# Zhang-Xin-Duke/multimodal-detection-consistency

Measured on AMD Instinct MI355X. Metric: defended queries/sec, higher is better.
Workload: dtype bf16; 1 GPU; ViT-L/14 bf16, batch=512/GPU, N=8 variants, 1000000-row bf16 bank, encode + exact top-5 bank search + consistency (BASELINE configs[2]); global_batch=512, parallelism=dp1, text_packing=eot-packed + variant prefix sharing (bit-identical, see DESIGN.md), bank=gaussian + planted neighbours of the text rows

## Files before the change

### include/tvc.h

```cpp
#ifndef TVC_H_
#define TVC_H_

#include <stdint.h>

#ifdef __cplusplus
extern "C" {
#endif

#define TVC_ABI_VERSION 4
#define TVC_MAX_BANKS 8
#define TVC_MAX_TOPK 128

enum {
    TVC_OK = 0,
    TVC_E_INVALID = 1,
    TVC_E_HIP = 2,
    TVC_E_NOMEM = 3,
    TVC_E_STATE = 4,
    TVC_E_OVERFLOW = 5
};

enum { TVC_DTYPE_BF16 = 0, TVC_DTYPE_F32 = 1 };

typedef struct tvc_handle tvc_handle;
// ... 97 lines not shown
int tvc_encode_image(tvc_handle* h, const float* pix_dev, int32_t B,
                     float* out_dev, int32_t normalize, void* stream);

int tvc_encode_text(tvc_handle* h, const int32_t* tok_dev, int32_t T,
                    float* out_dev, int32_t normalize, void* stream);


int tvc_bank_select(tvc_handle* h, int32_t slot);

int tvc_bank_set(tvc_handle* h, const void* bank_dev, int64_t R, int32_t D,
                 int32_t dtype, void* stream);

int tvc_bank_search(tvc_handle* h, const float* rows_dev, int32_t M, int32_t k,
                    float count_thr, int64_t idx_offset,
                    int32_t* topk_idx_dev, float* topk_sim_dev, float* moments_dev,
                    void* stream);

int tvc_bank_search_dense(tvc_handle* h, const float* rows_dev, int32_t M, int32_t k,
                          float count_thr, int64_t idx_offset,
                          int32_t* topk_idx_dev, float* topk_sim_dev, float* moments_dev,
                          void* stream);

int tvc_bank_status(tvc_handle* h, void* stream);

int tvc_bank_gather(tvc_handle* h, const int32_t* idx_dev, int32_t n,
                    int64_t idx_offset, float* out_dev, void* stream);

int tvc_topk_merge(tvc_handle* h, const int32_t* idx_parts_dev, const float* sim_parts_dev,
                   const float* feat_parts_dev, const float* mom_parts_dev,
                   int32_t W, int32_t M, int32_t k, int32_t kf, int32_t D,
                   int32_t* idx_out_dev, float* sim_out_dev, float* feat_out_dev,
                   float* mom_out_dev, void* stream);



int tvc_kmeans_assign(tvc_handle* h, const float* centroids_dev, int32_t K,
                      int32_t* labels_dev, float* score_dev, float* dist2_dev, void* stream);

int tvc_kmeans_update(tvc_handle* h, const int32_t* labels_dev, const float* centroids_in_dev, int32_t K,
                      float* centroids_out_dev, int32_t* counts_dev, int32_t* offsets_dev, int32_t* order_dev,
                      void* stream);


#define TVC_RADIUS_MAX_ROWS 131072

int tvc_radius_graph(tvc_handle* h, float eps, uint32_t* adj_dev, int32_t* degree_dev, void* stream);
// ... 203 lines not shown
```

### multimodal-detection-consistency_amd/_lib.py

```python
from __future__ import annotations

import ctypes as C
import os
import subprocess
import threading
from pathlib import Path

PKG_DIR = Path(__file__).resolve().parent
CSRC_DIR = PKG_DIR / "csrc"
LIB_PATH = Path(os.environ["TVC_LIB_PATH"]) if os.environ.get("TVC_LIB_PATH") else PKG_DIR / "libtvc_hip.so"
HEADER_PATH = PKG_DIR.parent / "include" / "tvc.h"

TVC_OK, TVC_E_INVALID, TVC_E_HIP, TVC_E_NOMEM, TVC_E_STATE, TVC_E_OVERFLOW = range(6)
TVC_DTYPE_BF16, TVC_DTYPE_F32 = 0, 1
TVC_REC_HEAD, TVC_REC_MAXREF = 12, 16
TVC_ABI_VERSION, TVC_MAX_BANKS, TVC_MAX_TOPK = 4, 8, 128
TVC_OPT_TEXT_PACKING, TVC_OPT_MAX_CHUNK_IMAGES, TVC_OPT_MAX_CHUNK_TEXTS, TVC_OPT_BANK_FILTER = 1, 2, 3, 4
TVC_OPT_TEXT_GROUP = 5
TVC_OPT_POOLED_LAST_LAYER = 6
TVC_OPT_TOWER_PRECISION = 7
TVC_OPT_SD_ARENA_BYTES = 8
TVC_OPT_SD_STREAMS = 9
TVC_OPT_SD_PRECISION = 10
TVC_OPT_GRAD_PRECISION = 11
# ... 72 lines not shown

TOWER_OPS = {name: code for code, name in enumerate((
    "layernorm", "layernorm_bwd", "lnpre_bwd", "assemble_lnpre", "im2col", "im2col_f32", "col2im", "gelu_fwd", "gelu_bwd",
    "gelu_erf_16", "gelu_erf_f32", "l2norm_rows", "l2norm_bwd", "ln_split", "rows_split", "split_planes", "gather_rows",
    "gather_f32_rows", "text_lens_scan", "text_embed"))}

GRAD_SPLIT_OPS = {name: code for code, name in enumerate(("gelu_bwd", "l2norm_bwd", "lnpre_bwd", "rows_split_t", "layernorm_bwd"))}


SIGNATURES = {
    "tvc_abi_version": (C.c_uint32, []),
    "tvc_create": (C.c_int, [C.POINTER(ModelDesc), C.POINTER(VisionWeights), C.POINTER(TextWeights), C.POINTER(_P)]),
    "tvc_destroy": (None, [_P]),
    "tvc_last_error": (C.c_char_p, [_P]),
    "tvc_workspace_bytes": (C.c_uint64, [_P]),
    "tvc_set_option": (C.c_int, [_P, C.c_int32, C.c_int64]),
    "tvc_encode_image": (C.c_int, [_P, _P, C.c_int32, _P, C.c_int32, _P]),
    "tvc_encode_text": (C.c_int, [_P, _P, C.c_int32, _P, C.c_int32, _P]),
    "tvc_bank_set": (C.c_int, [_P, _P, C.c_int64, C.c_int32, C.c_int32, _P]),
    "tvc_bank_select": (C.c_int, [_P, C.c_int32]),
    "tvc_bank_search": (C.c_int, [_P, _P, C.c_int32, C.c_int32, C.c_float, C.c_int64, _P, _P, _P, _P]),
    "tvc_bank_search_dense": (C.c_int, [_P, _P, C.c_int32, C.c_int32, C.c_float, C.c_int64, _P, _P, _P, _P]),
    "tvc_bank_status": (C.c_int, [_P, _P]),
    "tvc_bank_gather": (C.c_int, [_P, _P, C.c_int32, C.c_int64, _P, _P]),
    "tvc_kmeans_assign": (C.c_int, [_P, _P, C.c_int32, _P, _P, _P, _P]),
    "tvc_kmeans_update": (C.c_int, [_P, _P, _P, C.c_int32, _P, _P, _P, _P, _P]),
    "tvc_radius_graph": (C.c_int, [_P, C.c_float, _P, _P, _P]),
    "tvc_dbscan_sweep": (C.c_int, [_P, _P, _P, C.c_int32, C.c_int32, _P, _P, C.c_int32, _P]),
    "tvc_dbscan_finish": (C.c_int, [_P, _P, _P, C.c_int32, C.c_int32, _P, _P, _P, _P, _P]),
    "tvc_graph_pair_count": (C.c_int, [_P, _P, C.c_int32, _P, _P, _P]),
    "tvc_graph_pair_fill": (C.c_int, [_P, _P, C.c_int32, _P, _P, _P, C.c_int64, _P]),
    "tvc_pair_cosine": (C.c_int, [_P, _P, C.c_int64, _P, _P]),
    "tvc_ivf_probe": (C.c_int, [_P, _P, C.c_int32, C.c_int32, _P, C.c_int32, C.c_int32, _P, _P, _P]),
    "tvc_ivf_scan": (C.c_int, [_P, _P, C.c_int32, C.c_int32, _P, C.c_int32, _P, C.c_int32, C.c_int32, _P, C.c_int64, _P, _P, _P, _P]),
    "tvc_topk_merge": (C.c_int, [_P, _P, _P, _P, _P, C.c_int32, C.c_int32, C.c_int32, C.c_int32, C.c_int32,
                                 _P, _P, _P, _P, _P]),
    "tvc_cosine_matrix": (C.c_int, [_P, _P, C.c_int32, _P, C.c_int32, C.c_int32, _P, _P]),
    "tvc_consistency": (C.c_int, [_P, _P, _P, C.c_int32, C.c_int32, C.c_int32, _P, _P, _P, C.c_int32, C.c_int32,
                                  C.POINTER(ConsistencyParams), _P, _P]),
    "tvc_profile_begin": (C.c_int, [_P]),
    "tvc_profile_end": (C.c_int, [_P, C.POINTER(C.c_double), C.POINTER(C.c_double), C.POINTER(C.c_int64), _P]),
    "tvc_gemm_bf16": (C.c_int, [_P, _P, _P, _P, _P, C.c_int32, C.c_int32, C.c_int32, C.c_int64, C.c_int64, C.c_int32,
                                C.c_int32, _P]),
    "tvc_attention": (C.c_int, [_P, _P, _P, C.c_int32, C.c_int32, C.c_int32, C.c_int32, _P]),
    "tvc_layernorm": (C.c_int, [_P, _P, _P, _P, _P, C.c_int32, C.c_int32, _P]),
    "tvc_encode_text_hidden": (C.c_int, [_P, _P, C.c_int32, _P, _P]),
# ... 83 lines not shown
```

### multimodal-detection-consistency_amd/csrc/bank.hip

```cpp
#include "gemm_core.hpp"
#include "gemm_ring4.hpp"
#include "skinny.hpp"
#include "kernels.hpp"
#include "launch.hpp"
#include "select.hpp"
#include <cstdlib>

#define BANK_POOL 6144
#define BANK_MAX_RESCORE_D 2048
#define BANK_LDS_BYTES (GEMM_LDS_BYTES + 256 * 4 + 2 * 256 * 4 * 4)

struct Cand {
    float v;
    int32_t idx;
};

struct Moments {
    float sum = 0.f, sq = 0.f, mx = -INFINITY, cnt = 0.f;
};
__device__ __forceinline__ Moments combine(const Moments a, const Moments b) {
    Moments r;
    r.sum = a.sum + b.sum; r.sq = a.sq + b.sq; r.mx = fmaxf(a.mx, b.mx); r.cnt = a.cnt + b.cnt;
    return r;
}
__device__ __forceinline__ Moments mom_load(const float* p) {
    Moments r;
    r.sum = p[0]; r.sq = p[1]; r.mx = p[2]; r.cnt = p[3];
    return r;
}
__device__ __forceinline__ void mom_store(float* p, const Moments m) { p[0] = m.sum; p[1] = m.sq; p[2] = m.mx; p[3] = m.cnt; }
template <int... Os>
__device__ __forceinline__ Moments mom_lanes(Moments m) {
    ((m.sum += __shfl_xor(m.sum, Os, 64)), ...);
    ((m.sq += __shfl_xor(m.sq, Os, 64)), ...);
    ((m.cnt += __shfl_xor(m.cnt, Os, 64)), ...);
    ((m.mx = fmaxf(m.mx, __shfl_xor(m.mx, Os, 64))), ...);
    return m;
}


__device__ __forceinline__ void kth_finish(float m, int q, int k, float* __restrict__ tau, const uint16_t* __restrict__ qplanes,
                                           int D, const float* __restrict__ bank_bounds, float* gm, float (*nrm)[4]) {
    const int t = threadIdx.x;
    float margin = 0.f;
    if (qplanes) {
        float h2 = 0.f, l2 = 0.f;
        if (t < 256) {
            const uint16_t* qr = qplanes + (int64_t)q * 2 * D;
            for (int c = t; c < D; c += 256) {
                const float h = bf16_bits_to_f32(qr[c]), l = bf16_bits_to_f32(qr[D + c]);
                h2 = fmaf(h, h, h2); l2 = fmaf(l, l, l2);
            }
            h2 = wave_sum(h2); l2 = wave_sum(l2);
            if ((t & 63) == 0) { nrm[0][t >> 6] = h2; nrm[1][t >> 6] = l2; }
        }
        __syncthreads();
        const float qh = sqrtf(nrm[0][0] + nrm[0][1] + nrm[0][2] + nrm[0][3]);
        const float ql = sqrtf(nrm[1][0] + nrm[1][1] + nrm[1][2] + nrm[1][3]);
        const float bh = bank_bounds[0], bl = bank_bounds[1];
        margin = (bh * ql + bl * qh + bl * ql) * 1.001f + 4e-6f * (1.f + bh * qh);
    }
    if (t < 256) gm[t] = m;
    __syncthreads();
    if (t >= 256) return;
    int rank = 0;
    for (int u = 0; u < 256; ++u) {
        const float o = gm[u];
        rank += (o > m) || (o == m && u < t);
    }
    const int keff = k > BANK_KEFF ? k : BANK_KEFF;
    if (rank == keff - 1) {
        float v = m;
        if (v > -INFINITY) v = v - 1e-6f - 1e-6f * fabsf(v) - margin;
        if (!(v == v)) v = -INFINITY;
        tau[q] = v;
    }
}

__global__ __launch_bounds__(1024) void kth_bound_kernel(const float* __restrict__ s0, int n_sample,
                                                         int k, float* __restrict__ tau,
                                                         const uint16_t* __restrict__ qplanes, int D,
                                                         const float* __restrict__ bank_bounds) {
    __shared__ float gm[256];
    __shared__ float part[3][256];
    __shared__ float nrm[2][4];
    const int q = blockIdx.x, t = threadIdx.x;
    const float* row = s0 + (int64_t)q * n_sample;
    float m = -INFINITY;
    if ((n_sample & 3) == 0) {
        const f32x4_t* row4 = (const f32x4_t*)row;
        const int n4 = n_sample >> 2;
        int i = t;
        for (; i + 3 * 1024 < n4; i += 4 * 1024) {
            const f32x4_t a = row4[i], b = row4[i + 1024], c = row4[i + 2048], d = row4[i + 3072];
            m = fmaxf(m, fmaxf(fmaxf(fmaxf(a[0], a[1]), fmaxf(a[2], a[3])), fmaxf(fmaxf(b[0], b[1]), fmaxf(b[2], b[3]))));
            m = fmaxf(m, fmaxf(fmaxf(fmaxf(c[0], c[1]), fmaxf(c[2], c[3])), fmaxf(fmaxf(d[0], d[1]), fmaxf(d[2], d[3]))));
        }
        for (; i < n4; i += 1024) {
            const f32x4_t a = row4[i];
            m = fmaxf(m, fmaxf(fmaxf(a[0], a[1]), fmaxf(a[2], a[3])));
        }
    } else {
        for (int i = t; i < n_sample; i += 1024) m = fmaxf(m, row[i]);
    }
    if (t >= 256) part[(t >> 8) - 1][t & 255] = m;
    __syncthreads();
    if (t < 256) m = fmaxf(fmaxf(m, part[0][t]), fmaxf(part[1][t], part[2][t]));
    kth_finish(m, q, k, tau, qplanes, D, bank_bounds, gm, nrm);
}

__global__ __launch_bounds__(256) void kth_groups_kernel(const float* __restrict__ gmax, int k, float* __restrict__ tau,
                                                         const uint16_t* __restrict__ qplanes, int D,
                                                         const float* __restrict__ bank_bounds, int32_t* __restrict__ overflow) {
    __shared__ float gm[256];
    __shared__ float nrm[2][4];
    const int q = blockIdx.x;
    if (q == 0 && threadIdx.x == 0) *overflow = 0;
    kth_finish(gmax[(int64_t)q * 256 + threadIdx.x], q, k, tau, qplanes, D, bank_bounds, gm, nrm);
}

__global__ __launch_bounds__(256) void bank_bounds_kernel(BankRows bank, uint32_t* __restrict__ out_sq) {
    const int lane = threadIdx.x & 63, D = bank.D;
    float mh = 0.f, ml = 0.f;
    for (int64_t r = (int64_t)blockIdx.x * 4 + (threadIdx.x >> 6); r < bank.R; r += (int64_t)gridDim.x * 4) {
        const uint16_t* br = bank.p + r * bank.ld;
        float h2 = 0.f, l2 = 0.f;
        for (int c = lane * 8; c < D; c += 512) {
            const u32x4_t h = *(const u32x4_t*)(br + c);
#pragma unroll
            for (int e = 0; e < 4; ++e) {
                const float a = Op16<false>::lo(h[e]), b = Op16<false>::hi(h[e]);
                h2 = fmaf(a, a, fmaf(b, b, h2));
            }
            if (bank.planes > 1) {
                const u32x4_t l = *(const u32x4_t*)(br + D + c);
#pragma unroll
                for (int e = 0; e < 4; ++e) {
                    const float a = Op16<false>::lo(l[e]), b = Op16<false>::hi(l[e]);
                    l2 = fmaf(a, a, fmaf(b, b, l2));
                }
            }
// ... 342 lines not shown

template <int KB>
static hipError_t launch_sample_skinny_kb(const uint16_t* bank, int64_t ldb, const uint16_t* qplanes, int M, int n_sample,
                                          int sample_stride, float* gmax, hipStream_t stream) {
    const int nqt = M <= 16 ? 1 : (M > 32 && M <= 48) ? 3 : 2;
    const int per = (n_sample + 255) / 256;
    const dim3 grid(256, (M + nqt * 16 - 1) / (nqt * 16));
    const size_t lds = (size_t)nqt * 16 * (KB * 256 + 16) + 8 * nqt * 16 * 4;
    return dispatch<1, 2, 3>(nqt, [&](auto n) {
        constexpr size_t max_lds = n.value * 16 * (KB * 256 + 16) + 8 * n.value * 16 * 4;
        return launch<bank_sample_skinny_kernel<KB, n.value>, max_lds>(grid, dim3(512), lds, stream, bank, ldb, qplanes, M, n_sample,
                                                                       sample_stride, per, gmax);
    });
}
static hipError_t launch_bank_sample_skinny(const uint16_t* bank, int64_t ldb, int D, const uint16_t* qplanes, int M, int n_sample,
                                            int sample_stride, float* gmax, hipStream_t stream) {
    return dispatch<128, 512, 768>(D, [&](auto d) {
        return launch_sample_skinny_kb<d.value / 64>(bank, ldb, qplanes, M, n_sample, sample_stride, gmax, stream);
    });
}

#define SEL_T 1024
#define SEL_W (SEL_T / 64)
#define SEL_CPT 8
__global__ __launch_bounds__(SEL_T) void bank_select_kernel(const Cand* __restrict__ cand,
                                                            const int32_t* __restrict__ cand_cnt,
                                                            const float* __restrict__ mom_part, int S, int M,
                                                            int k, int32_t* __restrict__ topk_idx,
                                                            float* __restrict__ topk_sim,
                                                            float* __restrict__ moments,
                                                            int32_t* __restrict__ overflow, BankRows rs,
                                                            const float* __restrict__ rs_rows,
                                                            int64_t idx_offset) {
    __shared__ Cand pool[BANK_POOL];
    __shared__ __attribute__((aligned(16))) float qs[BANK_MAX_RESCORE_D];
    __shared__ int wsum[SEL_W];
    __shared__ BestSlots<SEL_T, 1> red;
    __shared__ float mom_red[SEL_W][4];
    const int q = blockIdx.x, t = threadIdx.x, D = rs.D;
    const int lane = t & 63, wave = t >> 6;

    const bool few = S <= SEL_T * SEL_CPT;
    int cnt[SEL_CPT];
    int mine = 0;
    if (few) {
#pragma unroll
        for (int u = 0; u < SEL_CPT; ++u) {
            const int c = t + u * SEL_T;
            cnt[u] = c < S ? cand_cnt[(int64_t)c * M + q] : 0;
        }
#pragma unroll
        for (int u = 0; u < SEL_CPT; ++u) mine += cnt[u];
    } else {
        for (int c = t; c < S; c += SEL_T) mine += cand_cnt[(int64_t)c * M + q];
    }
    int total_all;
    int off = block_exclusive_scan<SEL_T>(mine, wsum, total_all);
    if (few) {
#pragma unroll
        for (int u = 0; u < SEL_CPT; ++u) {
            const int n = cnt[u];
            if (n > 0) {
                const Cand* src = cand + ((int64_t)(t + u * SEL_T) * M + q) * BANK_CAP;
                for (int i = 0; i < n; ++i) {
                    if (off < BANK_POOL) pool[off] = src[i];
                    ++off;
                }
            }
        }
    } else {
        for (int c = t; c < S; c += SEL_T) {
            const int n = cand_cnt[(int64_t)c * M + q];
            const Cand* src = cand + ((int64_t)c * M + q) * BANK_CAP;
            for (int i = 0; i < n; ++i) {
                if (off < BANK_POOL) pool[off] = src[i];
                ++off;
            }
        }
    }
    if (t == 0 && total_all > BANK_POOL) atomicOr(overflow, 2);
    const int total = total_all < BANK_POOL ? total_all : BANK_POOL;
    if (rs.p) {
        for (int c = t; c < D; c += SEL_T) qs[c] = rs_rows[(int64_t)q * D + c];
    }
    __syncthreads();

    if (rs.p) {
        for (int i0 = wave; i0 < total; i0 += 4 * SEL_W) {
            float part[4];
            const uint16_t* br[4];
#pragma unroll
            for (int u = 0; u < 4; ++u) {
                int i = i0 + u * SEL_W;
                i = i < total ? i : total - 1;
                br[u] = rs.p + ((int64_t)pool[i].idx - idx_offset) * rs.ld;
                part[u] = 0.f;
            }
            for (int c = lane * 8; c < D; c += 512) {
                u32x4_t h[4], l[4];
#pragma unroll
                for (int u = 0; u < 4; ++u) {
                    h[u] = *(const u32x4_t*)(br[u] + c);
                    if (rs.planes > 1) l[u] = *(const u32x4_t*)(br[u] + D + c);
                }
                const f32x4_t q0 = *(const f32x4_t*)(qs + c), q1 = *(const f32x4_t*)(qs + c + 4);
#pragma unroll
                for (int u = 0; u < 4; ++u) {
#pragma unroll
                    for (int e2 = 0; e2 < 4; ++e2) {
                        float a = Op16<false>::lo(h[u][e2]), b = Op16<false>::hi(h[u][e2]);
                        if (rs.planes > 1) {
                            a += Op16<false>::lo(l[u][e2]);
                            b += Op16<false>::hi(l[u][e2]);
                        }
                        const float qa = e2 < 2 ? q0[e2 * 2] : q1[e2 * 2 - 4];
                        const float qb = e2 < 2 ? q0[e2 * 2 + 1] : q1[e2 * 2 - 3];
                        part[u] = fmaf(a, qa, fmaf(b, qb, part[u]));
                    }
                }
            }
#pragma unroll
            for (int u = 0; u < 4; ++u) {
                const float v = wave_sum(part[u]);
                const int i = i0 + u * SEL_W;
                if (lane == 0 && i < total) pool[i].v = v;
            }
        }
        __syncthreads();
    }

    for (int r = 0; r < k; ++r) {
        Best<1> b;
        b.pay[0] = -1;
        for (int i = t; i < total; i += SEL_T) {
            const Cand c = pool[i];
            if (c.idx >= 0) best_take(b, Best<1>{c.v, c.idx, {i}});
        }
        const Best<1> f = block_best(b, red, r);
        const int fp = f.pay[0];
        if (t == 0) {
            topk_idx[(int64_t)q * k + r] = fp >= 0 ? f.id : -1;
            topk_sim[(int64_t)q * k + r] = fp >= 0 ? f.v : -INFINITY;
        }
        if (fp >= 0 && (fp & (SEL_T - 1)) == t) pool[fp].idx = -1;
    }

    if (moments) {
        Moments m;
        for (int ch = t; ch < S; ch += SEL_T) m = combine(m, mom_load(mom_part + ((int64_t)ch * M + q) * 4));
        m = mom_lanes<32, 16, 8, 4, 2, 1>(m);
        if (lane == 0) mom_store(mom_red[wave], m);
        __syncthreads();
        if (t == 0) {
            Moments o;
            for (int w = 0; w < SEL_W; ++w) o = combine(o, mom_load(mom_red[w]));
            mom_store(moments + (int64_t)q * 4, o);
        }
// ... 52 lines not shown
        if (st != hipSuccess) return st;
    }
    return hipSuccess;
}

static bool env_flag(const char* name) {
    const char* v = getenv(name);
    return !v || atoi(v) != 0;
}

hipError_t launch_bank_search(const BankSearchLaunch& L, hipStream_t stream) {
    const BankRows& B = L.bank;
    const int D = B.D;
    const bool filter = (L.moments == nullptr) && L.bank_bounds && L.rows && D <= BANK_MAX_RESCORE_D && L.allow_filter;

    static const bool skinny_on = env_flag("TVC_BANK_SKINNY");
    const bool skinny = filter && skinny_on && skinny_covers(D, L.M) && B.ld % 8 == 0;
    static const bool skinny_sample_on = env_flag("TVC_BANK_SKINNY_SAMPLE");

    hipError_t st;
    if (skinny && skinny_sample_on && B.planes == 1) {
        st = launch_bank_sample_skinny(B.p, B.ld, D, L.qplanes, L.M, L.n_sample, L.sample_stride, L.gmax, stream);
        if (st != hipSuccess) return st;
        st = launch<kth_groups_kernel>(dim3(L.M), dim3(256), 0, stream, L.gmax, L.k, L.tau, L.qplanes, D, L.bank_bounds, L.overflow);
        if (st != hipSuccess) return st;
    } else {
        const GemmLaunch G = gemm_launch_planes(B.p, B.ld * (int64_t)L.sample_stride, L.n_sample, B.planes, L.qplanes, L.M, D,
                                                L.s0, L.n_sample);
        st = launch_gemm_bf16(G, stream);
        if (st != hipSuccess) return st;
        st = launch<kth_bound_kernel>(dim3(L.M), dim3(1024), 0, stream, L.s0, L.n_sample, L.k, L.tau, filter ? L.qplanes : nullptr, D,
                                      L.bank_bounds);
        if (st != hipSuccess) return st;
        st = hipMemsetAsync(L.overflow, 0, sizeof(int32_t), stream);
        if (st != hipSuccess) return st;
    }

    GemmOperands g = gemm_operands(gemm_launch_planes(B.p, B.ld, (int)B.R, B.planes, L.qplanes, L.M, D, nullptr, 0));
    if (filter) g.planes = 1;
    BankEpilogue e;
    e.tau = L.tau; e.cand = (Cand*)L.cand; e.cand_cnt = L.cand_cnt; e.mom_part = L.mom_part;
    e.overflow = L.overflow; e.R = B.R; e.idx_offset = L.idx_offset; e.M = L.M; e.count_thr = L.count_thr;
    const int nQt = (L.M + GEMM_BN - 1) / GEMM_BN;
    const int nbt = (int)((B.R + GEMM_BM - 1) / GEMM_BM);
    const int tpc = (nbt + L.S - 1) / L.S;
    static const bool ring_on = env_flag("TVC_BANK_RING");
    const bool ring = filter && ring_on && L.q_rows_padded && (g.lda % 64 == 0) && (g.ldb % 64 == 0) && B.R >= GEMM_BM;
    const dim3 grid(nQt * L.S), block(GEMM_THREADS);
    if (skinny)
        st = launch_bank_filter_skinny(B.p, B.ld, D, L.qplanes, e, L.S, tpc * GEMM_BM, stream);
    else if (ring)
        st = launch<bank_filter_ring_kernel, BANK_LDS_BYTES>(grid, block, BANK_LDS_BYTES, stream, g, e, nQt, L.S, tpc, nbt);
    else
        st = dispatch<false, true>(filter, [&](auto f) {
            return launch<bank_search_kernel<f.value>, BANK_LDS_BYTES>(grid, block, BANK_LDS_BYTES, stream, g, e, nQt, L.S, tpc, nbt);
        });
    if (st != hipSuccess) return st;

    BankRows rs = B;
    if (!filter) rs.p = nullptr;
    return launch<bank_select_kernel>(dim3(L.M), dim3(SEL_T), 0, stream, (const Cand*)L.cand, L.cand_cnt, L.mom_part, L.S, L.M, L.k,
                                      L.topk_idx, L.topk_sim, L.moments, L.overflow, rs, L.rows, L.idx_offset);
}

__global__ __launch_bounds__(256) void topk_merge_kernel(const int32_t* __restrict__ idx_parts,
                                                         const float* __restrict__ sim_parts,
                                                         const float* __restrict__ feat_parts,
                                                         const float* __restrict__ mom_parts, int W,
                                                         int M, int k, int kf, int D,
                                                         int32_t* __restrict__ idx_out,
                                                         float* __restrict__ sim_out,
                                                         float* __restrict__ feat_out,
                                                         float* __restrict__ mom_out) {
    __shared__ float sv[256];
    __shared__ int si[256];
    __shared__ int src_of_rank[32];
    const int q = blockIdx.x, t = threadIdx.x;
    const int n = W * k;
    float v = -INFINITY;
    int id = -1;
    if (t < n) {
        const int w = t / k, j = t - w * k;
        id = idx_parts[((int64_t)w * M + q) * k + j];
        v = (id >= 0) ? sim_parts[((int64_t)w * M + q) * k + j] : -INFINITY;
    }
// ... 56 lines not shown
```

### multimodal-detection-consistency_amd/csrc/handle.hpp

```cpp
#pragma once
#include "../../include/tvc.h"
#include "kernels.hpp"

#include <hip/hip_runtime.h>
#include <cstdio>
#include <cstring>
#include <string>
#include <vector>

inline thread_local std::string g_create_error;

enum Slot {
    WS_X = 0, WS_H, WS_QKV, WS_MLP, WS_CLS, WS_DELTA, WS_DELTA2, WS_SPLITK, WS_POOL, WS_TOWER_N,
    WS_TX = WS_TOWER_N, WS_TH, WS_TQKV, WS_TMLP, WS_TCLS, WS_TDELTA, WS_TDELTA2, WS_TSPLITK, WS_TPOOL,
    WS_PATCH, WS_EOT, WS_STARTS, WS_PFX, WS_LENS,
    WS_COSX, WS_COSY, WS_COSXP, WS_COSYP,
    WS_QPLANES, WS_S0, WS_TAU, WS_CAND, WS_CAND_CNT, WS_MOM_PART, WS_OVERFLOW,
    WS_GSAVE, WS_GOUT, WS_GXL, WS_GDX, WS_G16, WS_GMLP2, WS_GDQKV, WS_GSTATS, WS_GSMALL, WS_GPATCH,
    WS_PX, WS_PH, WS_PQKV, WS_PMLP, WS_PCLS, WS_P_N_END,
    WS_PTX = WS_P_N_END, WS_PTH, WS_PTQKV, WS_PTMLP, WS_PTCLS,
    WS_SX, WS_SH, WS_SQKV, WS_SU, WS_SM, WS_SDELTA1, WS_SDELTA2, WS_SCLS, WS_S_END,
    WS_STX = WS_S_END, WS_STH, WS_STQKV, WS_STU, WS_STM, WS_STDELTA1, WS_STDELTA2, WS_STCLS,
    WS_SD0, WS_SD1, WS_SD2, WS_SD3, WS_SD4, WS_SD5, WS_SD6, WS_SD7,
    WS_KM_CPLANES, WS_KM_HALFNORM, WS_KM_BLKCNT, WS_KM_OFFSETS, WS_KM_ORDER,
    WS_IVF_CPLANES, WS_IVF_PQPLANES, WS_IVF_HALFNORM, WS_IVF_SIMS,
    WS_IVF_QPLANES, WS_IVF_BLKCNT, WS_IVF_PCOUNTS, WS_IVF_POFFSETS, WS_IVF_PORDER, WS_IVF_SCORES,
    WS_GS_KEEP, WS_GS_GP, WS_GS_MP, WS_GS_WIDE, WS_GS_ROW, WS_GS_SMALL,
    WS_DB_NORM2, WS_DB_HALF,
    WS_COUNT
};

struct Buf {
    void* p = nullptr;
    size_t n = 0;
};

struct BankSlot {
    const uint16_t* bank = nullptr;
    void* owned = nullptr;
    int64_t R = 0;
// ... 19 lines not shown
    int gI = 0, gJ = 0, gK = 0, gP = 0, gS = 0;
};

template <class W, class L>
struct TowerWeights {
    W w{};
    std::vector<L> layers;
    bool set = false;
    void assign(const W& src, int n_layers) {
        w = src;
        layers.assign(src.layers, src.layers + n_layers);
        w.layers = layers.data();
        set = true;
    }
};

struct tvc_handle {
    tvc_model_desc desc{};
    TowerWeights<tvc_vision_weights, tvc_layer_weights> vision;
    TowerWeights<tvc_text_weights, tvc_layer_weights> text;
    BankSlot banks[TVC_MAX_BANKS];
    int cur_bank = 0;
    bool bank_filter = true;
    Buf ws[WS_COUNT];
    std::string err;
    int max_chunk_images = 512;
    int max_chunk_texts = 4608;
    bool pack_text = true;
    int text_group = 0;
    bool pooled_last = true;
    std::vector<void*> wT;
    int grad_B = 0;
    int grad_normalize = 0;
    const float* grad_pix = nullptr;
    int grad_precision = 0;
    int grad_mode = 0;
    bool prof = false;
    std::vector<ProfRec> prof_recs;
    TowerWeights<tvc_vision_weights_f32, tvc_layer_weights_f32> vision32;
    TowerWeights<tvc_text_weights_f32, tvc_layer_weights_f32> text32;
    int tower_precision = 0;
    TowerWeights<tvc_vision_weights, tvc_layer_weights> vision16;
    TowerWeights<tvc_text_weights, tvc_layer_weights> text16;
    std::vector<SplitLayer> vsplit, tsplit;
    uint16_t* vsplit_patch = nullptr;
    std::vector<void*> split_owned;
// ... 119 lines not shown
```

### multimodal-detection-consistency_amd/csrc/kernels.hpp

```cpp
#pragma once
#include <hip/hip_runtime.h>
#include <stdint.h>
#include "host_plan.hpp"

struct BankRows {
    const uint16_t* p = nullptr;
    int64_t ld = 0;
    int64_t R = 0;
    int D = 0;
    int planes = 1;
};

enum { TVC_EPI_F32 = 0, TVC_EPI_BF16 = 1, TVC_EPI_GELU_BF16 = 2, TVC_EPI_RESID_F32 = 3 };

struct GemmLaunch {
    const uint16_t* A = nullptr;
    const uint16_t* B = nullptr;
    int64_t lda = 0, ldb = 0;
    int I = 0, J = 0, K = 0;
    int planes = 1;
    int a_plane_off[9] = {0, 0, 0, 0, 0, 0, 0, 0, 0};
    int b_plane_off[9] = {0, 0, 0, 0, 0, 0, 0, 0, 0};
    bool splitk_small = false;
    int splitk_fixed = 0;
// ... 53 lines not shown
hipError_t launch_split_planes(const float* x, uint16_t* out, int64_t rows, int d, int planes,
                               hipStream_t stream);
hipError_t launch_gather_rows(const BankRows& bank, const int32_t* idx, int64_t idx_offset, int n, float* out, hipStream_t stream);

hipError_t launch_attention(const uint16_t* qkv, uint16_t* out, const int32_t* starts, int n_seq,
                            int seq_len, int heads, int causal, hipStream_t stream, const int32_t* pfx = nullptr,
                            int pool_mode = 0, const int32_t* pool_row = nullptr,
                            int f16 = 0);

struct BankSearchLaunch {
    BankRows bank;
    const uint16_t* qplanes = nullptr;
    const float* rows = nullptr;
    const float* bank_bounds = nullptr;
    bool allow_filter = true;
    bool q_rows_padded = false;
    int M = 0;
    int k = 0;
    float count_thr = 0.f;
    int64_t idx_offset = 0;
    float* s0 = nullptr;
    float* gmax = nullptr;
    float* tau = nullptr;
    void* cand = nullptr;
    int32_t* cand_cnt = nullptr;
    float* mom_part = nullptr;
    int32_t* overflow = nullptr;
    int n_sample = 0, sample_stride = 1, S = 0, cap = 0;
    int32_t* topk_idx = nullptr;
    float* topk_sim = nullptr;
    float* moments = nullptr;
};
hipError_t launch_bank_search(const BankSearchLaunch& L, hipStream_t stream);
hipError_t launch_bank_bounds(const BankRows& bank, float* bounds, hipStream_t stream);
hipError_t launch_bank_search_dense(const BankSearchLaunch& L, float* sims_ws, int block_rows, hipStream_t stream);
hipError_t launch_topk_merge(const int32_t* idx_parts, const float* sim_parts, const float* feat_parts,
                             const float* mom_parts, int W, int M, int k, int kf, int D,
                             int32_t* idx_out, float* sim_out, float* feat_out, float* mom_out,
                             hipStream_t stream);

struct KmeansAssignLaunch {
    BankRows bank;
    const float* centroids = nullptr;
    const uint16_t* cplanes = nullptr;
    int K = 0;
    float* halfnorm = nullptr;
// ... 172 lines not shown
```

### multimodal-detection-consistency_amd/csrc/tvc_abi.cpp

```cpp
#include "handle.hpp"

#include <cstdlib>

namespace {

bool tower_ok(const tvc_tower_arch& a) {
    return a.width > 0 && a.layers > 0 && a.heads > 0 && a.width == a.heads * 64 && a.width % 64 == 0 &&
           a.width <= 1024 && a.mlp > 0 && a.mlp % 64 == 0 && (a.act == TVC_ACT_QUICK_GELU || a.act == TVC_ACT_GELU);
}

struct PoolBufs { uint16_t *Hc, *D1c, *H2c, *MLPc, *D2c; };
PoolBufs pool_bufs(tvc_handle* h, const tvc_tower_arch& a, int n_seq, int wso) {
    uint16_t* p = (uint16_t*)h->ws[WS_POOL + wso].p;
    const size_t nd = ((size_t)n_seq + 256) * a.width;
    PoolBufs b;
    b.Hc = p; b.D1c = p + nd; b.H2c = p + 2 * nd; b.D2c = p + 3 * nd; b.MLPc = p + 4 * nd;
    return b;
}
size_t pool_bytes(const tvc_tower_arch& a, int n_seq) {
    return (((size_t)n_seq + 256) * a.width * 4 + ((size_t)n_seq + 256) * a.mlp) * 2;
}

struct GradSave {
    float* x;
// ... 378 lines not shown
                    int64_t idx_offset, int32_t* topk_idx_dev, float* topk_sim_dev, float* moments_dev,
                    void* stream) {
    if (!h) return TVC_E_INVALID;
    BankSlot& bk = h->banks[h->cur_bank];
    if (!bk.bank && bk.R != 0) return fail(h, TVC_E_STATE, "tvc_bank_search: no bank registered");
    if (bk.D == 0) return fail(h, TVC_E_STATE, "tvc_bank_search: call tvc_bank_set first");
    if (M < 0 || k < 1 || k > TVC_MAX_TOPK || (M > 0 && (!rows_dev || !topk_idx_dev || !topk_sim_dev)))
        return fail(h, TVC_E_INVALID, "tvc_bank_search: need 1 <= k <= 128 and non-NULL buffers");
    if (M == 0) return TVC_OK;
    hipStream_t st = (hipStream_t)stream;
    const int D = bk.D;
    if (bk.R == 0) {
        HIP_TRY(hipMemsetAsync(topk_idx_dev, 0xff, (size_t)M * k * 4, st));
        HIP_TRY(hipMemsetAsync(topk_sim_dev, 0, (size_t)M * k * 4, st));
        if (moments_dev) HIP_TRY(hipMemsetAsync(moments_dev, 0, (size_t)M * 16, st));
        return TVC_OK;
    }
    BankSearchLaunch L;
    bank_plan(bk.R, M, k, &L.n_sample, &L.sample_stride, &L.S, &L.cap);
    int rc;
    if ((rc = ensure(h, WS_QPLANES, (size_t)((M + 255) / 256 * 256) * 2 * D * 2))) return rc;
    if ((rc = ensure(h, WS_S0, (size_t)M * (L.n_sample > 256 ? L.n_sample : 256) * 4))) return rc;
    if ((rc = ensure(h, WS_TAU, (size_t)M * 4))) return rc;
    if ((rc = ensure(h, WS_CAND, (size_t)L.S * M * L.cap * 8))) return rc;
    if ((rc = ensure(h, WS_CAND_CNT, (size_t)L.S * M * 4))) return rc;
    if ((rc = ensure(h, WS_MOM_PART, (size_t)L.S * M * 16))) return rc;
    if ((rc = ensure(h, WS_OVERFLOW, 16))) return rc;
    HIP_TRY(launch_split_planes(rows_dev, (uint16_t*)h->ws[WS_QPLANES].p, M, D, 2, st));
    L.bank = bank_rows(bk);
    L.qplanes = (const uint16_t*)h->ws[WS_QPLANES].p; L.q_rows_padded = true; L.M = M; L.k = k; L.count_thr = count_thr;
    L.idx_offset = idx_offset;
    L.rows = rows_dev; L.bank_bounds = bk.bounds; L.allow_filter = h->bank_filter;
    L.s0 = (float*)h->ws[WS_S0].p; L.gmax = L.s0; L.tau = (float*)h->ws[WS_TAU].p; L.cand = h->ws[WS_CAND].p;
    L.cand_cnt = (int32_t*)h->ws[WS_CAND_CNT].p; L.mom_part = (float*)h->ws[WS_MOM_PART].p;
    L.overflow = (int32_t*)h->ws[WS_OVERFLOW].p;
    L.topk_idx = topk_idx_dev; L.topk_sim = topk_sim_dev; L.moments = moments_dev;
    {
        const bool filter = !moments_dev && h->bank_filter && D <= 2048;
        const int planes = filter ? 1 : bank_products(bk.planes);
        ProfScope ps(h, st, TVC_PROF_BANK, 2.0 * (double)bk.R * M * D * planes);
        HIP_TRY(launch_bank_search(L, st));
    }
    return TVC_OK;
}

int tvc_bank_search_dense(tvc_handle* h, const float* rows_dev, int32_t M, int32_t k, float count_thr,
                          int64_t idx_offset, int32_t* topk_idx_dev, float* topk_sim_dev, float* moments_dev,
                          void* stream) {
    if (!h) return TVC_E_INVALID;
    BankSlot& bk = h->banks[h->cur_bank];
    if (bk.D == 0 || (!bk.bank && bk.R != 0)) return fail(h, TVC_E_STATE, "tvc_bank_search_dense: call tvc_bank_set first");
    if (M < 0 || k < 1 || k > TVC_MAX_TOPK || (M > 0 && (!rows_dev || !topk_idx_dev || !topk_sim_dev)))
        return fail(h, TVC_E_INVALID, "tvc_bank_search_dense: need 1 <= k <= 128 and non-NULL buffers");
    if (M == 0) return TVC_OK;
    if (bk.R == 0) return tvc_bank_search(h, rows_dev, M, k, count_thr, idx_offset, topk_idx_dev, topk_sim_dev, moments_dev, stream);
    hipStream_t st = (hipStream_t)stream;
    const int D = bk.D;
    int block = (int)((size_t)1 << 28) / (int)(bk.R > 0 ? bk.R : 1);
    if (block > 64) block = 64;
    if (block < 1) block = 1;
    int rc;
    if ((rc = ensure(h, WS_QPLANES, (size_t)((M + 255) / 256 * 256) * 2 * D * 2))) return rc;
    if ((rc = ensure(h, WS_S0, (size_t)block * bk.R * 4))) return rc;
    HIP_TRY(launch_split_planes(rows_dev, (uint16_t*)h->ws[WS_QPLANES].p, M, D, 2, st));
    BankSearchLaunch L;
// ... 280 lines not shown
                           int32_t seq_len, int32_t heads, void* stream) {
    if (!h) return TVC_E_INVALID;
    if (!qkv_dev || !dout_dev || !dqkv_dev) return fail(h, TVC_E_INVALID, "tvc_attention_backward: NULL buffer");
    if (n_seq < 0 || seq_len < 0 || heads < 0)
        return fail(h, TVC_E_INVALID, "tvc_attention_backward: n_seq, seq_len and heads must not be negative");
    int rc;
    if ((rc = ensure(h, WS_GSTATS, (size_t)n_seq * seq_len * heads * 16))) return rc;
    HIP_TRY(launch_attention_bwd(qkv_dev, dout_dev, dqkv_dev, (float*)h->ws[WS_GSTATS].p, n_seq, seq_len, heads, (hipStream_t)stream));
    return TVC_OK;
}

int tvc_layernorm_backward(tvc_handle* h, const float* x_dev, const uint16_t* dy_dev, const float* g_dev, const float* dres_dev,
                           float* dx_dev, int32_t rows, int32_t d, void* stream) {
    if (!h) return TVC_E_INVALID;
    if (!x_dev || !dy_dev || !g_dev || !dx_dev) return fail(h, TVC_E_INVALID, "tvc_layernorm_backward: NULL buffer");
    HIP_TRY(launch_layernorm_bwd(x_dev, d, nullptr, dy_dev, 0, g_dev, dres_dev, dx_dev, nullptr, rows, d, d, (hipStream_t)stream));
    return TVC_OK;
}

int tvc_set_option(tvc_handle* h, int32_t option, int64_t value) {
    if (!h) return TVC_E_INVALID;
    switch (option) {
        case TVC_OPT_TEXT_PACKING: h->pack_text = value != 0; return TVC_OK;
        case TVC_OPT_BANK_FILTER: h->bank_filter = value != 0; return TVC_OK;
        case TVC_OPT_POOLED_LAST_LAYER: h->pooled_last = value != 0; return TVC_OK;
        case TVC_OPT_TOWER_PRECISION: {
            if (value < 0 || value > 3)
                return fail(h, TVC_E_INVALID, "tvc_set_option: TVC_OPT_TOWER_PRECISION must be 0 (bf16), 1 (fp32), 2 (split-bf16) or 3 (fp16)");
            if (value == 3) {
                if (!h->vision16.set && !h->text16.set)
                    return fail(h, TVC_E_INVALID, "tvc_set_option: TVC_OPT_TOWER_PRECISION = 3 needs tvc_set_weights_f16 first");
                h->tower_precision = 3; return TVC_OK;
            }
            if (value != 0 && !h->vision32.set && !h->text32.set)
                return fail(h, TVC_E_STATE, "tvc_set_option: TVC_OPT_TOWER_PRECISION = 1 / 2 needs tvc_set_weights_f32 first");
            if (value == 2) {
                const int rc = tvc_split_prepare(h);
                if (rc) return rc;
            }
            h->tower_precision = (int)value; return TVC_OK;
        }
        case TVC_OPT_GRAD_PRECISION:
            if (value != 0 && value != 2)
                return fail(h, TVC_E_INVALID, "tvc_set_option: TVC_OPT_GRAD_PRECISION must be 0 (bf16) or 2 (split-bf16)");
            if (value == 2 && h->vision32.set) {
                const int rc = tvc_split_prepare(h);
                if (rc) return rc;
// ... 168 lines not shown
```

### multimodal-detection-consistency_amd/engine.py

```python
from __future__ import annotations

import contextlib
import ctypes as C
import threading
from dataclasses import dataclass, field
from typing import Dict, Optional, Tuple

import torch

from . import _lib
from .arch import ClipArch


@dataclass
class ConsistencyConfig:
    reference_count: int = 5
    similarity_threshold: float = 0.3
    retrieval_top_k: int = 10
    dup_threshold: float = 0.95
    w_text_variants: float = 0.4
    w_consistency: float = 0.2
    w_exp: Tuple[float, float, float, float] = (0.25, 0.25, 0.25, 0.25)
    search_k: int = 5

# ... 439 lines not shown
        self.dense_fallbacks += 1
        return out

    def bank_search_dense(self, rows: torch.Tensor, k: int, count_thr: float = 0.3, idx_offset: int = 0,
                          want_moments: bool = True, bank: str = DEFAULT_BANK, out=None):
        if not 1 <= k <= _lib.TVC_MAX_TOPK:
            raise ValueError(f"top-k must be in [1, {_lib.TVC_MAX_TOPK}] (got {k})")
        rows = _require_cuda(rows, torch.float32, "rows")
        M = rows.shape[0]
        if out is None:
            out = (torch.empty((M, k), dtype=torch.int32, device=self.device),
                   torch.empty((M, k), dtype=torch.float32, device=self.device),
                   torch.empty((M, 4), dtype=torch.float32, device=self.device) if want_moments else None)
        idx, sim, mom = out
        with self._lock, torch.cuda.device(self.device):
            self._select(bank)
            self._check(self.lib.tvc_bank_search_dense(self.handle, _ptr(rows), M, k, count_thr, idx_offset,
                                                       _ptr(idx), _ptr(sim), _ptr(mom), _stream()))
        return idx, sim, mom

    def bank_status(self) -> None:
        with self._lock, torch.cuda.device(self.device):
            self._check(self.lib.tvc_bank_status(self.handle, _stream()))

    def bank_gather(self, idx: torch.Tensor, idx_offset: int = 0, bank: str = DEFAULT_BANK) -> torch.Tensor:
        idx = _require_cuda(idx, torch.int32, "idx")
        n = idx.numel()
        with self._lock, torch.cuda.device(self.device):
            b = self._select(bank)
            out = torch.empty((n, b["dim"]), dtype=torch.float32, device=self.device)
            self._check(self.lib.tvc_bank_gather(self.handle, _ptr(idx), n, idx_offset, _ptr(out), _stream()))
        return out.view(*idx.shape, b["dim"])

    def kmeans_assign(self, centroids: torch.Tensor, bank: str = DEFAULT_BANK):
        centroids = _require_cuda(centroids, torch.float32, "centroids")
        with self._lock, torch.cuda.device(self.device):
            b = self._select(bank)
            if centroids.dim() != 2 or centroids.shape[1] != b["dim"]:
                raise ValueError(f"centroids must be [K, {b['dim']}] (got {tuple(centroids.shape)})")
            R = b["rows"]
            labels = torch.empty(R, dtype=torch.int32, device=self.device)
            score = torch.empty(R, dtype=torch.float32, device=self.device)
            dist2 = torch.empty(R, dtype=torch.float32, device=self.device)
            self._check(self.lib.tvc_kmeans_assign(self.handle, _ptr(centroids), centroids.shape[0], _ptr(labels), _ptr(score),
                                                   _ptr(dist2), _stream()))
        return labels, score, dist2
# ... 587 lines not shown
```

Baseline: 5305 queries/s.

## Prune rescore candidates with a bounded error band before exact bank rescoring

The select kernel now finds the approximate k-th best score in the candidate pool. It then drops every candidate whose approximate score falls below that value minus an error band built from the per-query quantisation margin and bf16 rounding slack, and compacts the pool before the exact two-plane rescore. The aim is to cut the global bank-row reads and dot products spent in the rescore pass. In exchange it adds k block-wide reductions, a scan, and new margin and live-count buffers, along with a debug API to read the live counts. Rows per rescore iteration drop from 4 to 2, with an occupancy hint in launch bounds.

```diff
diff --git a/include/tvc.h b/include/tvc.h
--- a/include/tvc.h
+++ b/include/tvc.h
@@ -143,6 +143,8 @@
                           void* stream);
 
 int tvc_bank_status(tvc_handle* h, void* stream);
+
+int tvc_bank_live_counts(tvc_handle* h, int32_t* out_dev, int32_t M, void* stream);
 
 int tvc_bank_gather(tvc_handle* h, const int32_t* idx_dev, int32_t n,
                     int64_t idx_offset, float* out_dev, void* stream);
diff --git a/multimodal-detection-consistency_amd/_lib.py b/multimodal-detection-consistency_amd/_lib.py
--- a/multimodal-detection-consistency_amd/_lib.py
+++ b/multimodal-detection-consistency_amd/_lib.py
@@ -118,6 +118,7 @@
     "tvc_bank_search": (C.c_int, [_P, _P, C.c_int32, C.c_int32, C.c_float, C.c_int64, _P, _P, _P, _P]),
     "tvc_bank_search_dense": (C.c_int, [_P, _P, C.c_int32, C.c_int32, C.c_float, C.c_int64, _P, _P, _P, _P]),
     "tvc_bank_status": (C.c_int, [_P, _P]),
+    "tvc_bank_live_counts": (C.c_int, [_P, _P, C.c_int32, _P]),
     "tvc_bank_gather": (C.c_int, [_P, _P, C.c_int32, C.c_int64, _P, _P]),
     "tvc_kmeans_assign": (C.c_int, [_P, _P, C.c_int32, _P, _P, _P, _P]),
     "tvc_kmeans_update": (C.c_int, [_P, _P, _P, C.c_int32, _P, _P, _P, _P, _P]),
diff --git a/multimodal-detection-consistency_amd/csrc/bank.hip b/multimodal-detection-consistency_amd/csrc/bank.hip
--- a/multimodal-detection-consistency_amd/csrc/bank.hip
+++ b/multimodal-detection-consistency_amd/csrc/bank.hip
@@ -40,7 +40,8 @@
 
 
 __device__ __forceinline__ void kth_finish(float m, int q, int k, float* __restrict__ tau, const uint16_t* __restrict__ qplanes,
-                                           int D, const float* __restrict__ bank_bounds, float* gm, float (*nrm)[4]) {
+                                           int D, const float* __restrict__ bank_bounds, float* gm, float (*nrm)[4],
+                                           float* __restrict__ margin_out) {
     const int t = threadIdx.x;
     float margin = 0.f;
     if (qplanes) {
@@ -59,6 +60,7 @@
         const float ql = sqrtf(nrm[1][0] + nrm[1][1] + nrm[1][2] + nrm[1][3]);
         const float bh = bank_bounds[0], bl = bank_bounds[1];
         margin = (bh * ql + bl * qh + bl * ql) * 1.001f + 4e-6f * (1.f + bh * qh);
+        if (t == 0 && margin_out) margin_out[q] = margin;
     }
     if (t < 256) gm[t] = m;
     __syncthreads();
@@ -80,7 +82,7 @@
 __global__ __launch_bounds__(1024) void kth_bound_kernel(const float* __restrict__ s0, int n_sample,
                                                          int k, float* __restrict__ tau,
                                                          const uint16_t* __restrict__ qplanes, int D,
-                                                         const float* __restrict__ bank_bounds) {
+                                                         const float* __restrict__ bank_bounds, float* __restrict__ margin_out) {
     __shared__ float gm[256];
     __shared__ float part[3][256];
     __shared__ float nrm[2][4];
@@ -106,17 +108,18 @@
     if (t >= 256) part[(t >> 8) - 1][t & 255] = m;
     __syncthreads();
     if (t < 256) m = fmaxf(fmaxf(m, part[0][t]), fmaxf(part[1][t], part[2][t]));
-    kth_finish(m, q, k, tau, qplanes, D, bank_bounds, gm, nrm);
+    kth_finish(m, q, k, tau, qplanes, D, bank_bounds, gm, nrm, margin_out);
 }
 
 __global__ __launch_bounds__(256) void kth_groups_kernel(const float* __restrict__ gmax, int k, float* __restrict__ tau,
                                                          const uint16_t* __restrict__ qplanes, int D,
-                                                         const float* __restrict__ bank_bounds, int32_t* __restrict__ overflow) {
+                                                         const float* __restrict__ bank_bounds, int32_t* __restrict__ overflow,
+                                                         float* __restrict__ margin_out) {
     __shared__ float gm[256];
     __shared__ float nrm[2][4];
     const int q = blockIdx.x;
     if (q == 0 && threadIdx.x == 0) *overflow = 0;
-    kth_finish(gmax[(int64_t)q * 256 + threadIdx.x], q, k, tau, qplanes, D, bank_bounds, gm, nrm);
+    kth_finish(gmax[(int64_t)q * 256 + threadIdx.x], q, k, tau, qplanes, D, bank_bounds, gm, nrm, margin_out);
 }
 
 __global__ __launch_bounds__(256) void bank_bounds_kernel(BankRows bank, uint32_t* __restrict__ out_sq) {
@@ -505,8 +508,11 @@
 
 #define SEL_T 1024
 #define SEL_W (SEL_T / 64)
-#define SEL_CPT 8
-__global__ __launch_bounds__(SEL_T) void bank_select_kernel(const Cand* __restrict__ cand,
+#define SEL_ROWS 2
+#define SEL_CPT 2
+#define SEL_OWN (BANK_POOL / SEL_T)
+static_assert(SEL_OWN * SEL_T == BANK_POOL && (SEL_T & (SEL_T - 1)) == 0, "the pool is dealt evenly to the threads");
+__global__ __launch_bounds__(SEL_T, 8) void bank_select_kernel(const Cand* __restrict__ cand,
                                                             const int32_t* __restrict__ cand_cnt,
                                                             const float* __restrict__ mom_part, int S, int M,
                                                             int k, int32_t* __restrict__ topk_idx,
@@ -514,10 +520,13 @@
                                                             float* __restrict__ moments,
                                                             int32_t* __restrict__ overflow, BankRows rs,
                                                             const float* __restrict__ rs_rows,
-                                                            int64_t idx_offset) {
+                                                            int64_t idx_offset, const float* __restrict__ margin,
+                                                            const float* __restrict__ bank_bounds,
+                                                            int32_t* __restrict__ live_out) {
     __shared__ Cand pool[BANK_POOL];
     __shared__ __attribute__((aligned(16))) float qs[BANK_MAX_RESCORE_D];
     __shared__ int wsum[SEL_W];
+    __shared__ float qn2[SEL_W];
     __shared__ BestSlots<SEL_T, 1> red;
     __shared__ float mom_red[SEL_W][4];
     const int q = blockIdx.x, t = threadIdx.x, D = rs.D;
@@ -564,31 +573,86 @@
     if (t == 0 && total_all > BANK_POOL) atomicOr(overflow, 2);
     const int total = total_all < BANK_POOL ? total_all : BANK_POOL;
     if (rs.p) {
-        for (int c = t; c < D; c += SEL_T) qs[c] = rs_rows[(int64_t)q * D + c];
-    }
-    __syncthreads();
+        float q2 = 0.f;
+        for (int c = t; c < D; c += SEL_T) {
+            const float x = rs_rows[(int64_t)q * D + c];
+            qs[c] = x;
+            q2 = fmaf(x, x, q2);
+        }
+        q2 = wave_sum(q2);
+        if (lane == 0) qn2[wave] = q2;
+    }
+    __syncthreads();
+
+    int n_live = total;
+    if (rs.p && margin) {
+        float qn = 0.f;
+#pragma unroll
+        for (int w = 0; w < SEL_W; ++w) qn += qn2[w];
+        qn = sqrtf(qn);
+        const float slack = 1.01f * (3.f * (float)D * 5.9604645e-8f + 3.0517578e-5f) * (bank_bounds[0] + bank_bounds[1]) * qn;
+        const float band = 2.f * (margin[q] + slack);
+        bool prune = total_all <= BANK_POOL && total >= k && band < INFINITY;
+        Cand own[SEL_OWN];
+#pragma unroll
+        for (int j = 0; j < SEL_OWN; ++j) {
+            const int i = t + j * SEL_T;
+            own[j].v = -INFINITY; own[j].idx = -1;
+            if (i < total) own[j] = pool[i];
+        }
+        unsigned struck = 0u;
+        float L = 0.f;
+        for (int r = 0; prune && r < k; ++r) {
+            Best<1> b;
+            b.pay[0] = -1;
+#pragma unroll
+            for (int j = 0; j < SEL_OWN; ++j)
+                if (own[j].idx >= 0 && !((struck >> j) & 1u)) best_take(b, Best<1>{own[j].v, own[j].idx, {t + j * SEL_T}});
+            const Best<1> f = block_best(b, red, r);
+            const int fp = f.pay[0];
+            if (fp < 0) prune = false;
+            else if ((fp & (SEL_T - 1)) == t) struck |= 1u << (fp / SEL_T);
+            L = f.v;
+        }
+        if (prune) {
+            float thr = L - band;
+            thr -= 4.8e-7f * fabsf(thr);
+            int mine_live = 0;
+#pragma unroll
+            for (int j = 0; j < SEL_OWN; ++j) {
+                if (!(own[j].idx >= 0 && own[j].v >= thr)) own[j].idx = -1;
+                mine_live += own[j].idx >= 0 ? 1 : 0;
+            }
+            int at = block_exclusive_scan<SEL_T>(mine_live, wsum, n_live);
+#pragma unroll
+            for (int j = 0; j < SEL_OWN; ++j)
+                if (own[j].idx >= 0) pool[at++] = own[j];
+        }
+        __syncthreads();
+    }
+    if (live_out && t == 0) { live_out[2 * (int64_t)q] = n_live; live_out[2 * (int64_t)q + 1] = total; }
 
     if (rs.p) {
-        for (int i0 = wave; i0 < total; i0 += 4 * SEL_W) {
-            float part[4];
-            const uint16_t* br[4];
-#pragma unroll
-            for (int u = 0; u < 4; ++u) {
+        for (int i0 = wave; i0 < n_live; i0 += SEL_ROWS * SEL_W) {
+            float part[SEL_ROWS];
+            const uint16_t* br[SEL_ROWS];
+#pragma unroll
+            for (int u = 0; u < SEL_ROWS; ++u) {
                 int i = i0 + u * SEL_W;
-                i = i < total ? i : total - 1;
+                i = i < n_live ? i : n_live - 1;
                 br[u] = rs.p + ((int64_t)pool[i].idx - idx_offset) * rs.ld;
                 part[u] = 0.f;
             }
             for (int c = lane * 8; c < D; c += 512) {
-                u32x4_t h[4], l[4];
-#pragma unroll
-                for (int u = 0; u < 4; ++u) {
+                u32x4_t h[SEL_ROWS], l[SEL_ROWS];
+#pragma unroll
+                for (int u = 0; u < SEL_ROWS; ++u) {
                     h[u] = *(const u32x4_t*)(br[u] + c);
                     if (rs.planes > 1) l[u] = *(const u32x4_t*)(br[u] + D + c);
                 }
                 const f32x4_t q0 = *(const f32x4_t*)(qs + c), q1 = *(const f32x4_t*)(qs + c + 4);
 #pragma unroll
-                for (int u = 0; u < 4; ++u) {
+                for (int u = 0; u < SEL_ROWS; ++u) {
 #pragma unroll
                     for (int e2 = 0; e2 < 4; ++e2) {
                         float a = Op16<false>::lo(h[u][e2]), b = Op16<false>::hi(h[u][e2]);
@@ -603,10 +667,10 @@
                 }
             }
 #pragma unroll
-            for (int u = 0; u < 4; ++u) {
+            for (int u = 0; u < SEL_ROWS; ++u) {
                 const float v = wave_sum(part[u]);
                 const int i = i0 + u * SEL_W;
-                if (lane == 0 && i < total) pool[i].v = v;
+                if (lane == 0 && i < n_live) pool[i].v = v;
             }
         }
         __syncthreads();
@@ -615,7 +679,7 @@
     for (int r = 0; r < k; ++r) {
         Best<1> b;
         b.pay[0] = -1;
-        for (int i = t; i < total; i += SEL_T) {
+        for (int i = t; i < n_live; i += SEL_T) {
             const Cand c = pool[i];
             if (c.idx >= 0) best_take(b, Best<1>{c.v, c.idx, {i}});
         }
@@ -714,7 +778,8 @@
     if (skinny && skinny_sample_on && B.planes == 1) {
         st = launch_bank_sample_skinny(B.p, B.ld, D, L.qplanes, L.M, L.n_sample, L.sample_stride, L.gmax, stream);
         if (st != hipSuccess) return st;
-        st = launch<kth_groups_kernel>(dim3(L.M), dim3(256), 0, stream, L.gmax, L.k, L.tau, L.qplanes, D, L.bank_bounds, L.overflow);
+        st = launch<kth_groups_kernel>(dim3(L.M), dim3(256), 0, stream, L.gmax, L.k, L.tau, L.qplanes, D, L.bank_bounds, L.overflow,
+                                       L.margin);
         if (st != hipSuccess) return st;
     } else {
         const GemmLaunch G = gemm_launch_planes(B.p, B.ld * (int64_t)L.sample_stride, L.n_sample, B.planes, L.qplanes, L.M, D,
@@ -722,7 +787,7 @@
         st = launch_gemm_bf16(G, stream);
         if (st != hipSuccess) return st;
         st = launch<kth_bound_kernel>(dim3(L.M), dim3(1024), 0, stream, L.s0, L.n_sample, L.k, L.tau, filter ? L.qplanes : nullptr, D,
-                                      L.bank_bounds);
+                                      L.bank_bounds, L.margin);
         if (st != hipSuccess) return st;
         st = hipMemsetAsync(L.overflow, 0, sizeof(int32_t), stream);
         if (st != hipSuccess) return st;
@@ -751,8 +816,10 @@
 
     BankRows rs = B;
     if (!filter) rs.p = nullptr;
+    const float* margin = (filter && L.bounded_rescore) ? L.margin : nullptr;
     return launch<bank_select_kernel>(dim3(L.M), dim3(SEL_T), 0, stream, (const Cand*)L.cand, L.cand_cnt, L.mom_part, L.S, L.M, L.k,
-                                      L.topk_idx, L.topk_sim, L.moments, L.overflow, rs, L.rows, L.idx_offset);
+                                      L.topk_idx, L.topk_sim, L.moments, L.overflow, rs, L.rows, L.idx_offset, margin, L.bank_bounds,
+                                      L.live);
 }
 
 __global__ __launch_bounds__(256) void topk_merge_kernel(const int32_t* __restrict__ idx_parts,
diff --git a/multimodal-detection-consistency_amd/csrc/handle.hpp b/multimodal-detection-consistency_amd/csrc/handle.hpp
--- a/multimodal-detection-consistency_amd/csrc/handle.hpp
+++ b/multimodal-detection-consistency_amd/csrc/handle.hpp
@@ -15,7 +15,7 @@
     WS_TX = WS_TOWER_N, WS_TH, WS_TQKV, WS_TMLP, WS_TCLS, WS_TDELTA, WS_TDELTA2, WS_TSPLITK, WS_TPOOL,
     WS_PATCH, WS_EOT, WS_STARTS, WS_PFX, WS_LENS,
     WS_COSX, WS_COSY, WS_COSXP, WS_COSYP,
-    WS_QPLANES, WS_S0, WS_TAU, WS_CAND, WS_CAND_CNT, WS_MOM_PART, WS_OVERFLOW,
+    WS_QPLANES, WS_S0, WS_TAU, WS_MARGIN, WS_LIVE, WS_CAND, WS_CAND_CNT, WS_MOM_PART, WS_OVERFLOW,
     WS_GSAVE, WS_GOUT, WS_GXL, WS_GDX, WS_G16, WS_GMLP2, WS_GDQKV, WS_GSTATS, WS_GSMALL, WS_GPATCH,
     WS_PX, WS_PH, WS_PQKV, WS_PMLP, WS_PCLS, WS_P_N_END,
     WS_PTX = WS_P_N_END, WS_PTH, WS_PTQKV, WS_PTMLP, WS_PTCLS,
@@ -81,6 +81,8 @@
     BankSlot banks[TVC_MAX_BANKS];
     int cur_bank = 0;
     bool bank_filter = true;
+    bool bank_bounded = true;
+    int bank_live_rows = 0;
     Buf ws[WS_COUNT];
     std::string err;
     int max_chunk_images = 512;
diff --git a/multimodal-detection-consistency_amd/csrc/kernels.hpp b/multimodal-detection-consistency_amd/csrc/kernels.hpp
--- a/multimodal-detection-consistency_amd/csrc/kernels.hpp
+++ b/multimodal-detection-consistency_amd/csrc/kernels.hpp
@@ -99,6 +99,9 @@
     float* s0 = nullptr;
     float* gmax = nullptr;
     float* tau = nullptr;
+    float* margin = nullptr;
+    bool bounded_rescore = true;
+    int32_t* live = nullptr;
     void* cand = nullptr;
     int32_t* cand_cnt = nullptr;
     float* mom_part = nullptr;
diff --git a/multimodal-detection-consistency_amd/csrc/tvc_abi.cpp b/multimodal-detection-consistency_amd/csrc/tvc_abi.cpp
--- a/multimodal-detection-consistency_amd/csrc/tvc_abi.cpp
+++ b/multimodal-detection-consistency_amd/csrc/tvc_abi.cpp
@@ -424,6 +424,8 @@
     if ((rc = ensure(h, WS_QPLANES, (size_t)((M + 255) / 256 * 256) * 2 * D * 2))) return rc;
     if ((rc = ensure(h, WS_S0, (size_t)M * (L.n_sample > 256 ? L.n_sample : 256) * 4))) return rc;
     if ((rc = ensure(h, WS_TAU, (size_t)M * 4))) return rc;
+    if ((rc = ensure(h, WS_MARGIN, (size_t)M * 4))) return rc;
+    if ((rc = ensure(h, WS_LIVE, (size_t)M * 8))) return rc;
     if ((rc = ensure(h, WS_CAND, (size_t)L.S * M * L.cap * 8))) return rc;
     if ((rc = ensure(h, WS_CAND_CNT, (size_t)L.S * M * 4))) return rc;
     if ((rc = ensure(h, WS_MOM_PART, (size_t)L.S * M * 16))) return rc;
@@ -434,6 +436,7 @@
     L.idx_offset = idx_offset;
     L.rows = rows_dev; L.bank_bounds = bk.bounds; L.allow_filter = h->bank_filter;
     L.s0 = (float*)h->ws[WS_S0].p; L.gmax = L.s0; L.tau = (float*)h->ws[WS_TAU].p; L.cand = h->ws[WS_CAND].p;
+    L.margin = (float*)h->ws[WS_MARGIN].p; L.live = (int32_t*)h->ws[WS_LIVE].p; L.bounded_rescore = h->bank_bounded;
     L.cand_cnt = (int32_t*)h->ws[WS_CAND_CNT].p; L.mom_part = (float*)h->ws[WS_MOM_PART].p;
     L.overflow = (int32_t*)h->ws[WS_OVERFLOW].p;
     L.topk_idx = topk_idx_dev; L.topk_sim = topk_sim_dev; L.moments = moments_dev;
@@ -443,6 +446,17 @@
         ProfScope ps(h, st, TVC_PROF_BANK, 2.0 * (double)bk.R * M * D * planes);
         HIP_TRY(launch_bank_search(L, st));
     }
+    h->bank_live_rows = M;
+    return TVC_OK;
+}
+
+int tvc_bank_live_counts(tvc_handle* h, int32_t* out_dev, int32_t M, void* stream) {
+    if (!h) return TVC_E_INVALID;
+    if (M < 0 || (M > 0 && !out_dev)) return fail(h, TVC_E_INVALID, "tvc_bank_live_counts: bad arguments");
+    if (M > h->bank_live_rows || (M > 0 && !h->ws[WS_LIVE].p))
+        return fail(h, TVC_E_STATE, "tvc_bank_live_counts: the last tvc_bank_search on this handle had fewer query rows");
+    if (M == 0) return TVC_OK;
+    HIP_TRY(hipMemcpyAsync(out_dev, h->ws[WS_LIVE].p, (size_t)M * 8, hipMemcpyDeviceToDevice, (hipStream_t)stream));
     return TVC_OK;
 }
 
@@ -769,7 +783,7 @@
     if (!h) return TVC_E_INVALID;
     switch (option) {
         case TVC_OPT_TEXT_PACKING: h->pack_text = value != 0; return TVC_OK;
-        case TVC_OPT_BANK_FILTER: h->bank_filter = value != 0; return TVC_OK;
+        case TVC_OPT_BANK_FILTER: h->bank_filter = value != 0; h->bank_bounded = value != 2; return TVC_OK;
         case TVC_OPT_POOLED_LAST_LAYER: h->pooled_last = value != 0; return TVC_OK;
         case TVC_OPT_TOWER_PRECISION: {
             if (value < 0 || value > 3)
diff --git a/multimodal-detection-consistency_amd/engine.py b/multimodal-detection-consistency_amd/engine.py
--- a/multimodal-detection-consistency_amd/engine.py
+++ b/multimodal-detection-consistency_amd/engine.py
@@ -485,6 +485,12 @@
     def bank_status(self) -> None:
         with self._lock, torch.cuda.device(self.device):
             self._check(self.lib.tvc_bank_status(self.handle, _stream()))
+
+    def bank_live_counts(self, M: int) -> torch.Tensor:
+        out = torch.empty((M, 2), dtype=torch.int32, device=self.device)
+        with self._lock, torch.cuda.device(self.device):
+            self._check(self.lib.tvc_bank_live_counts(self.handle, _ptr(out), M, _stream()))
+        return out
 
     def bank_gather(self, idx: torch.Tensor, idx_offset: int = 0, bank: str = DEFAULT_BANK) -> torch.Tensor:
         idx = _require_cuda(idx, torch.int32, "idx")
```

New measurement: 5325 queries/s (median of 5 runs). Within noise of the previous version (+0.4%).
